# hzeller/timg

Measured on NVIDIA H100. Metric: Mpixels/s scale+dither+sixel-encode @4K→cell, higher is better.
Workload: dtype u8/f32

## Files before the change

### timg_b200/csrc/sixel_dither.cu

```cuda
#include <algorithm>
#include <cstdlib>

#include "sixel.cuh"

namespace b200timg {

#ifdef CUSIM
__device__ __forceinline__ uint32_t prmt(uint32_t a, uint32_t b, uint32_t s) { return __byte_perm(a, b, s); }
#else
__device__ __forceinline__ uint32_t prmt(uint32_t a, uint32_t b, uint32_t s) {
    uint32_t d;
    asm("prmt.b32 %0, %1, %2, %3;" : "=r"(d) : "r"(a), "r"(b), "r"(s));
    return d;
}
#endif

constexpr int D2_WMAX = 24;
constexpr int D2_CH = 16;
constexpr int D2_IN_STRIDE = D2_CH + 1;
constexpr int D2_OUT_STRIDE = 20;
constexpr int D2_WARP_SMEM = 2 * 32 * D2_IN_STRIDE * 4 + 32 * D2_OUT_STRIDE + D2_CH * 16;

struct TapW { uint32_t r, g, b; };

template <int K> __device__ __forceinline__ uint32_t tap_rg(const TapW &t) {
    constexpr uint32_t sel = (uint32_t)K | ((8u | K) << 4) | ((4u + K) << 8) | ((8u | (4u + K)) << 12);
    return prmt(t.r, t.g, sel);
}
template <int K> __device__ __forceinline__ uint32_t tap_b(const TapW &t) {
    constexpr uint32_t sel = (uint32_t)K | ((8u | K) << 4) | (4u << 8) | (4u << 12);
    return prmt(t.b, 0u, sel);
}
__device__ __forceinline__ uint32_t add_clamp(uint32_t v, uint32_t t) { return __viaddmin_s16x2_relu(v, t, 0x00ff00ffu); }

struct Dither2Geom { int w, h, nb32, bands_per_cta, nwarps; unsigned spin_ns; };

struct DitherUniform {
    typedef Dither2Geom Params;
    const Dither2Geom &G; int f, g;
    __device__ __forceinline__ explicit DitherUniform(const Dither2Geom &p) : G(p), f(blockIdx.y), g(blockIdx.x) {}
    __device__ __forceinline__ int w() const { return G.w; }
    __device__ __forceinline__ int h() const { return G.h; }
    __device__ __forceinline__ int nb32() const { return G.nb32; }
    __device__ __forceinline__ int bands_per_cta() const { return G.bands_per_cta; }
    __device__ __forceinline__ int nwarps() const { return G.nwarps; }
    __device__ __forceinline__ unsigned spin_ns() const { return G.spin_ns; }
    __device__ __forceinline__ long long px0() const { return (long long)f * G.w * G.h; }
    __device__ __forceinline__ long long idx0() const { return (long long)f * G.w * G.h; }
    __device__ __forceinline__ long long bnd0() const { return (long long)f * G.nb32 * G.w; }
    __device__ __forceinline__ long long prog0() const { return (long long)f * G.nb32; }
};
struct DitherMixed {
    typedef MixedSixelParams Params;
    MixedSixelFrame D; int f, g, nw;
    __device__ __forceinline__ explicit DitherMixed(const MixedSixelParams &P) : nw(P.nwarps) {
        f = sixel_owner(P.cta_start, P.n_frames, blockIdx.x);
        g = (int)(blockIdx.x - P.cta_start[f]);
        D = P.desc[f];
    }
    __device__ __forceinline__ int w() const { return D.w; }
    __device__ __forceinline__ int h() const { return D.h; }
    __device__ __forceinline__ int nb32() const { return D.nb32; }
    __device__ __forceinline__ int bands_per_cta() const { return D.bands_per_cta; }
    __device__ __forceinline__ int nwarps() const { return nw; }
    __device__ __forceinline__ unsigned spin_ns() const { return 256; }
    __device__ __forceinline__ long long px0() const { return (long long)D.fb_px; }
    __device__ __forceinline__ long long idx0() const { return (long long)D.idx; }
    __device__ __forceinline__ long long bnd0() const { return (long long)D.bnd; }
    __device__ __forceinline__ long long prog0() const { return (long long)D.prog0; }
};

template <class A>
__global__ void __launch_bounds__(D2_WMAX * 32)
sixel_dither2_kernel(const uint32_t *__restrict__ fb, typename A::Params G, SixelWork W, uint4 *__restrict__ bnd_all, int *__restrict__ gprog_all) {
    extern __shared__ __align__(16) uint8_t s_dyn2[];
    __shared__ uint2 s_pal2[256];
    __shared__ uint32_t s_tap[512];
    __shared__ volatile int s_progress[2048];
    const A a(G);
    const int f = a.f, g = a.g;
    const SixelFrameHdr *hdr = W.hdr + f;
    if (!hdr->diffuse) return;
    const int tid = threadIdx.x, lane = tid & 31, wid = tid >> 5;
    const int nthreads = a.nwarps() * 32, w = a.w(), h = a.h();
    uint8_t *s_lut = s_dyn2;
    for (int i = tid; i < 32768 / 16; i += nthreads)
        reinterpret_cast<uint4 *>(s_lut)[i] = reinterpret_cast<const uint4 *>(W.lut + (long long)f * 32768)[i];
    for (int i = tid; i < 256; i += nthreads) {
        const uint32_t p = hdr->palette[i];
        s_pal2[i] = make_uint2((256u - (p & 0xff)) | ((256u - ((p >> 8) & 0xff)) << 16), (256u - ((p >> 16) & 0xff)) | (256u << 16));
    }
    for (int i = tid; i < 512; i += nthreads) {
        const int e = i - 256;
        const int t7 = e * 7 / 16, t3 = e * 3 / 16, t5 = e * 5 / 16, t1 = e / 16;
        s_tap[i] = (uint32_t)(t7 & 0xff) | ((uint32_t)(t3 & 0xff) << 8) | ((uint32_t)(t5 & 0xff) << 16) | ((uint32_t)(t1 & 0xff) << 24);
    }
    const int band_lo = g * a.bands_per_cta(), band_hi = min(a.nb32(), band_lo + a.bands_per_cta());
    const int nlocal = band_hi - band_lo;
    for (int i = tid; i < nlocal; i += nthreads) s_progress[i] = 0;
    __syncthreads();
    uint32_t *s_in = reinterpret_cast<uint32_t *>(s_dyn2 + 32768 + (size_t)wid * D2_WARP_SMEM);
    uint8_t *s_out = reinterpret_cast<uint8_t *>(s_in + 2 * 32 * D2_IN_STRIDE);
    uint4 *s_bnd = reinterpret_cast<uint4 *>(s_out + 32 * D2_OUT_STRIDE);
    const uint32_t *frame = fb + a.px0();
    uint8_t *index = W.index + a.idx0();
    uint4 *bnd = bnd_all + a.bnd0();
    volatile int *gprog = gprog_all + a.prog0();
    const int hrow = lane >> 4, hcol = lane & 15;
    const int qrow = lane >> 3, qcol = lane & 7;
    const bool even_w = (w & 1) == 0;
    const TapW Z = {0u, 0u, 0u};

    for (int band = band_lo + wid; band < band_hi; band += a.nwarps()) {
        const int lb = band - band_lo;
        const int y = band * 32 + lane;
        const bool row_ok = y < h, last_row = (y == h - 1);
        const bool prev_remote = band > 0 && lb == 0;
        const bool publish_remote = band + 1 < a.nb32() && band + 1 == band_hi;
        const uint4 *bin = band > 0 ? bnd + (long long)(band - 1) * w : nullptr;
        uint4 *bout = bnd + (long long)band * w;
        TapW own = Z, a0 = Z, a1 = Z, a2 = Z, e_first = Z;
        const int steps = w + 62, nchunks = (steps + D2_CH - 1) / D2_CH;
        uint32_t pre[16];
        auto load_chunk = [&](int c) {
            if (even_w) {
#pragma unroll
                for (int i = 0; i < 8; ++i) {
                    const int r = 4 * i + qrow, yy = band * 32 + r, x = c * D2_CH - 2 * r + 2 * qcol;
                    uint2 v = make_uint2(0u, 0u);
                    if (yy < h && x >= 0 && x < w) v = *reinterpret_cast<const uint2 *>(frame + (long long)yy * w + x);
                    pre[2 * i] = v.x; pre[2 * i + 1] = v.y;
                }
            } else {
#pragma unroll
                for (int i = 0; i < 16; ++i) {
                    const int r = 2 * i + hrow, yy = band * 32 + r, x = c * D2_CH - 2 * r + hcol;
                    pre[i] = (yy < h && x >= 0 && x < w) ? frame[(long long)yy * w + x] : 0u;
                }
            }
        };
        auto store_chunk = [&](int c) {
            uint32_t *t = s_in + (c & 1) * 32 * D2_IN_STRIDE;
            if (even_w) {
#pragma unroll
                for (int i = 0; i < 8; ++i) {
                    uint32_t *q = t + (4 * i + qrow) * D2_IN_STRIDE + 2 * qcol;
                    q[0] = pre[2 * i]; q[1] = pre[2 * i + 1];
                }
            } else {
#pragma unroll
                for (int i = 0; i < 16; ++i) t[(2 * i + hrow) * D2_IN_STRIDE + hcol] = pre[i];
            }
        };
        load_chunk(0); store_chunk(0);
        __syncwarp();
        for (int c = 0; c < nchunks; ++c) {
            const int t0 = c * D2_CH;
            if (c + 1 < nchunks) load_chunk(c + 1);
            if (band > 0) {
                const int need = min(w, t0 + D2_CH + 1);
                if (lane == 0) {
                    if (prev_remote) { while (gprog[band - 1] < need) __nanosleep(a.spin_ns()); __threadfence(); }
                    else { while (s_progress[lb - 1] < need) __nanosleep(a.spin_ns()); __threadfence_block(); }
                }
                __syncwarp();
                const int bx = t0 + 1 + lane;
                if (lane < D2_CH) s_bnd[lane] = bx < w ? __ldcg(bin + bx) : make_uint4(0u, 0u, 0u, 0u);
                if (c == 0 && lane == 0) { const uint4 q = __ldcg(bin); a0.r = q.x; a0.g = q.y; a0.b = q.z; }
                __syncwarp();
            }
            const uint32_t *tin = s_in + (c & 1) * 32 * D2_IN_STRIDE + lane * D2_IN_STRIDE;
            const bool interior = (t0 - 62 >= 1) && (t0 + D2_CH - 1 <= w - 2) && (band * 32 + 31 < h - 1);
            if (interior) {
#pragma unroll 4
                for (int j = 0; j < D2_CH; ++j) {
                    TapW n;
                    n.r = __shfl_up_sync(0xffffffffu, own.r, 1); n.g = __shfl_up_sync(0xffffffffu, own.g, 1); n.b = __shfl_up_sync(0xffffffffu, own.b, 1);
                    if (lane == 0) { if (band > 0) { const uint4 q = s_bnd[j]; n.r = q.x; n.g = q.y; n.b = q.z; } else n = Z; }
                    a2 = a1; a1 = a0; a0 = n;
                    const uint32_t px = tin[j];
                    uint32_t vrg = prmt(px, 0u, 0x4140u), vb = prmt(px, 0u, 0x4442u);
                    vrg = add_clamp(vrg, tap_rg<3>(a2)); vb = add_clamp(vb, tap_b<3>(a2));
                    vrg = add_clamp(vrg, tap_rg<2>(a1)); vb = add_clamp(vb, tap_b<2>(a1));
                    vrg = add_clamp(vrg, tap_rg<1>(a0)); vb = add_clamp(vb, tap_b<1>(a0));
                    vrg = add_clamp(vrg, tap_rg<0>(own)); vb = add_clamp(vb, tap_b<0>(own));
                    const uint32_t cell = ((vrg & 0xf8u) << 7) | ((vrg >> 14) & 0x3e0u) | (vb >> 3);
                    const uint32_t ci = s_lut[cell];
                    const uint2 np = s_pal2[ci];
                    const uint32_t erg = vrg + np.x, eb = vb + np.y;
                    own.r = s_tap[erg & 0x1ffu]; own.g = s_tap[erg >> 16]; own.b = s_tap[eb & 0x1ffu];
                    s_out[lane * D2_OUT_STRIDE + j] = (uint8_t)ci;
                    if (lane == 31) __stcg(bout + (t0 + j - 62), make_uint4(own.r, own.g, own.b, 0u));
                }
            } else {
#pragma unroll 2
                for (int j = 0; j < D2_CH; ++j) {
                    const int t = t0 + j, x = t - 2 * lane;
                    TapW n;
                    n.r = __shfl_up_sync(0xffffffffu, own.r, 1); n.g = __shfl_up_sync(0xffffffffu, own.g, 1); n.b = __shfl_up_sync(0xffffffffu, own.b, 1);
                    if (lane == 0) { if (band > 0) { const uint4 q = s_bnd[j]; n.r = q.x; n.g = q.y; n.b = q.z; } else n = Z; }
                    a2 = a1; a1 = a0; a0 = n;
                    uint32_t ci = 0;
                    if (x >= 0 && x < w && row_ok) {
                        const uint32_t px = tin[j];
                        uint32_t vrg = prmt(px, 0u, 0x4140u), vb = prmt(px, 0u, 0x4442u);
                        vrg = add_clamp(vrg, tap_rg<3>(a2)); vb = add_clamp(vb, tap_b<3>(a2));
                        vrg = add_clamp(vrg, tap_rg<2>(a1)); vb = add_clamp(vb, tap_b<2>(a1));
                        vrg = add_clamp(vrg, tap_rg<1>(a0)); vb = add_clamp(vb, tap_b<1>(a0));
                        if (x == w - 1) { vrg = add_clamp(vrg, tap_rg<1>(e_first)); vb = add_clamp(vb, tap_b<1>(e_first)); }
                        vrg = add_clamp(vrg, tap_rg<0>(own)); vb = add_clamp(vb, tap_b<0>(own));
                        const uint32_t cell = ((vrg & 0xf8u) << 7) | ((vrg >> 14) & 0x3e0u) | (vb >> 3);
                        ci = s_lut[cell];
                        if (x < w - 1 && !last_row) {
                            const uint2 np = s_pal2[ci];
                            const uint32_t erg = vrg + np.x, eb = vb + np.y;
                            own.r = s_tap[erg & 0x1ffu]; own.g = s_tap[erg >> 16]; own.b = s_tap[eb & 0x1ffu];
                        } else {
                            own = Z;
                        }
                        if (x == 0) e_first = own;
                        if (lane == 31) __stcg(bout + x, make_uint4(own.r, own.g, own.b, 0u));
                    } else if (x >= w) {
                        own = Z;
                    }
                    s_out[lane * D2_OUT_STRIDE + j] = (uint8_t)ci;
                }
            }
            __syncwarp();
            if (even_w) {
#pragma unroll
                for (int i = 0; i < 8; ++i) {
                    const int r = 4 * i + qrow, yy = band * 32 + r, x = t0 - 2 * r + 2 * qcol;
                    if (yy < h && x >= 0 && x < w)
                        *reinterpret_cast<unsigned short *>(index + (long long)yy * w + x) =
                            *reinterpret_cast<const unsigned short *>(s_out + r * D2_OUT_STRIDE + 2 * qcol);
                }
            } else {
#pragma unroll
                for (int i = 0; i < 16; ++i) {
                    const int r = 2 * i + hrow, yy = band * 32 + r, x = t0 - 2 * r + hcol;
                    if (yy < h && x >= 0 && x < w) index[(long long)yy * w + x] = s_out[r * D2_OUT_STRIDE + hcol];
                }
            }
            {
                const int done = min(w, t0 + D2_CH - 62);
                if (lane == 31 && done > 0) {
                    if (publish_remote) { __threadfence(); gprog[band] = done; }
                    __threadfence_block();
                    s_progress[lb] = done;
                }
            }
            if (c + 1 < nchunks) store_chunk(c + 1);
            __syncwarp();
        }
    }
}

size_t sixel_dither_workspace(int w, int h, int n_frames, size_t *o_bnd, size_t *o_prog) {
    const size_t nb32 = (size_t)(h + 31) / 32;
    size_t off = 0;
    *o_bnd = off; off += (sizeof(uint4) * nb32 * (size_t)w * n_frames + 255) / 256 * 256;
    *o_prog = off; off += (sizeof(int) * nb32 * n_frames + 255) / 256 * 256;
    return off;
}

SixelDitherShape sixel_dither_shape(int nb32, int n_frames, int n_total, int sm_count, bool env) {
    SixelDitherShape S;
    int per_frame = 1;
    if (n_total < sm_count) {
        per_frame = std::max(1, std::min(sm_count / n_total, (nb32 + 7) / 8));
        if (const char *e = env ? getenv("B200TIMG_DITHER_SPLIT") : nullptr) per_frame = std::max(1, std::min(atoi(e), nb32));
        if ((long long)per_frame * n_frames > sm_count) per_frame = std::max(1, sm_count / n_frames);
    }
    S.bands_per_cta = (nb32 + per_frame - 1) / per_frame;
    S.per_frame = (nb32 + S.bands_per_cta - 1) / S.bands_per_cta;
    int wmax = D2_WMAX;
    if (const char *e = env ? getenv("B200TIMG_DITHER_WARPS") : nullptr) wmax = std::max(1, std::min(atoi(e), D2_WMAX));
    S.rounds = (S.bands_per_cta + wmax - 1) / wmax;
    S.nwarps = (S.bands_per_cta + S.rounds - 1) / S.rounds;
    return S;
}

int launch_sixel_dither(b200timg_ctx *ctx, const uint32_t *fb, int w, int h, int n_frames, int n_total, const SixelWork &W, void *d_bnd, void *d_prog) {
    Dither2Geom G;
    G.w = w; G.h = h; G.nb32 = (h + 31) / 32;
    G.spin_ns = 256;
    if (const char *e = getenv("B200TIMG_DITHER_SPIN")) G.spin_ns = (unsigned)std::max(0, std::min(atoi(e), 100000));
    const SixelDitherShape S = sixel_dither_shape(G.nb32, n_frames, n_total, ctx->sm_count, true);
    const int per_frame = S.per_frame;
    G.bands_per_cta = S.bands_per_cta;
    G.nwarps = S.nwarps;
    const size_t smem = 32768 + (size_t)G.nwarps * D2_WARP_SMEM;
    B2_CUDA(ctx, cudaFuncSetAttribute(sixel_dither2_kernel<DitherUniform>, cudaFuncAttributeMaxDynamicSharedMemorySize, 32768 + D2_WMAX * D2_WARP_SMEM));
    if (per_frame > 1) B2_CUDA(ctx, cudaMemsetAsync(d_prog, 0, sizeof(int) * (size_t)G.nb32 * n_frames, ctx->stream));
    B2_KERNEL(ctx, "sixel_dither2_kernel");
    sixel_dither2_kernel<DitherUniform><<<dim3(per_frame, n_frames), G.nwarps * 32, smem, ctx->stream>>>(fb, G, W, static_cast<uint4 *>(d_bnd), static_cast<int *>(d_prog));
    B2_LAUNCH_CHECK(ctx);
    return B200TIMG_OK;
}

int launch_sixel_dither_mixed(b200timg_ctx *ctx, const uint32_t *fb, unsigned n_ctas, const MixedSixelParams &M, const SixelWork &W,
                              void *d_bnd, void *d_prog, size_t n_prog, bool split) {
    const size_t smem = 32768 + (size_t)M.nwarps * D2_WARP_SMEM;
    B2_CUDA(ctx, cudaFuncSetAttribute(sixel_dither2_kernel<DitherMixed>, cudaFuncAttributeMaxDynamicSharedMemorySize, 32768 + D2_WMAX * D2_WARP_SMEM));
    if (split) B2_CUDA(ctx, cudaMemsetAsync(d_prog, 0, sizeof(int) * n_prog, ctx->stream));
    B2_KERNEL(ctx, "sixel_dither2_mixed_kernel");
    sixel_dither2_kernel<DitherMixed><<<n_ctas, M.nwarps * 32, smem, ctx->stream>>>(fb, M, W, static_cast<uint4 *>(d_bnd), static_cast<int *>(d_prog));
    B2_LAUNCH_CHECK(ctx);
    return B200TIMG_OK;
}

}
```

Baseline: 75790.

## Reorder dither chunk pipeline and stage boundary stores through shared memory

Moves the next-chunk global load after the neighbor-band wait. Lane 31 now stages boundary error terms in a per-warp shared buffer, and 16 lanes write them to global in one coalesced burst. The index write-back moves after progress publication, so downstream bands are unblocked sooner, and the interior loop packs four palette indices per 32-bit shared store. Palette and tap tables move into dynamic shared memory. Optional clock instrumentation is added behind a compile flag, at the cost of slightly more shared memory per warp.

```diff
diff --git a/timg_b200/csrc/sixel_dither.cu b/timg_b200/csrc/sixel_dither.cu
--- a/timg_b200/csrc/sixel_dither.cu
+++ b/timg_b200/csrc/sixel_dither.cu
@@ -19,7 +19,8 @@
 constexpr int D2_CH = 16;
 constexpr int D2_IN_STRIDE = D2_CH + 1;
 constexpr int D2_OUT_STRIDE = 20;
-constexpr int D2_WARP_SMEM = 2 * 32 * D2_IN_STRIDE * 4 + 32 * D2_OUT_STRIDE + D2_CH * 16;
+constexpr int D2_WARP_SMEM = 2 * 32 * D2_IN_STRIDE * 4 + 32 * D2_OUT_STRIDE + 2 * D2_CH * 16;
+constexpr int D2_TABLES = 32768 + 2048 + 2048;
 
 struct TapW { uint32_t r, g, b; };
 
@@ -32,6 +33,7 @@
     return prmt(t.b, 0u, sel);
 }
 __device__ __forceinline__ uint32_t add_clamp(uint32_t v, uint32_t t) { return __viaddmin_s16x2_relu(v, t, 0x00ff00ffu); }
+
 
 struct Dither2Geom { int w, h, nb32, bands_per_cta, nwarps; unsigned spin_ns; };
 
@@ -70,17 +72,33 @@
     __device__ __forceinline__ long long prog0() const { return (long long)D.prog0; }
 };
 
+#ifdef B200TIMG_DITHER_CLOCKS
+enum { DCLK_SETUP, DCLK_WAIT, DCLK_FETCH, DCLK_STEPS, DCLK_STAGE, DCLK_PHASES };
+__device__ unsigned long long g_dither_clocks[DCLK_PHASES + 1];
+#define DCLK_BEGIN unsigned dclk_[DCLK_PHASES] = {}, dclk_steps_ = 0; unsigned dclk_t_ = (unsigned)clock()
+#define DCLK(k) do { const unsigned t_ = (unsigned)clock(); dclk_[k] += t_ - dclk_t_; dclk_t_ = t_; } while (0)
+#define DCLK_STEP(n) (dclk_steps_ += (n))
+#define DCLK_END() do { if ((threadIdx.x & 31) == 0) { for (int k_ = 0; k_ < DCLK_PHASES; ++k_) \
+        atomicAdd(&g_dither_clocks[k_], (unsigned long long)dclk_[k_]); atomicAdd(&g_dither_clocks[DCLK_PHASES], (unsigned long long)dclk_steps_); } } while (0)
+#else
+#define DCLK_BEGIN do {} while (0)
+#define DCLK(k) do {} while (0)
+#define DCLK_STEP(n) do {} while (0)
+#define DCLK_END() do {} while (0)
+#endif
+
 template <class A>
 __global__ void __launch_bounds__(D2_WMAX * 32)
 sixel_dither2_kernel(const uint32_t *__restrict__ fb, typename A::Params G, SixelWork W, uint4 *__restrict__ bnd_all, int *__restrict__ gprog_all) {
     extern __shared__ __align__(16) uint8_t s_dyn2[];
-    __shared__ uint2 s_pal2[256];
-    __shared__ uint32_t s_tap[512];
+    uint2 *s_pal2 = reinterpret_cast<uint2 *>(s_dyn2 + 32768);
+    uint32_t *s_tap = reinterpret_cast<uint32_t *>(s_dyn2 + 32768 + 2048);
     __shared__ volatile int s_progress[2048];
     const A a(G);
     const int f = a.f, g = a.g;
     const SixelFrameHdr *hdr = W.hdr + f;
     if (!hdr->diffuse) return;
+    DCLK_BEGIN;
     const int tid = threadIdx.x, lane = tid & 31, wid = tid >> 5;
     const int nthreads = a.nwarps() * 32, w = a.w(), h = a.h();
     uint8_t *s_lut = s_dyn2;
@@ -99,9 +117,11 @@
     const int nlocal = band_hi - band_lo;
     for (int i = tid; i < nlocal; i += nthreads) s_progress[i] = 0;
     __syncthreads();
-    uint32_t *s_in = reinterpret_cast<uint32_t *>(s_dyn2 + 32768 + (size_t)wid * D2_WARP_SMEM);
+    DCLK(DCLK_SETUP);
+    uint32_t *s_in = reinterpret_cast<uint32_t *>(s_dyn2 + D2_TABLES + (size_t)wid * D2_WARP_SMEM);
     uint8_t *s_out = reinterpret_cast<uint8_t *>(s_in + 2 * 32 * D2_IN_STRIDE);
     uint4 *s_bnd = reinterpret_cast<uint4 *>(s_out + 32 * D2_OUT_STRIDE);
+    uint4 *s_bo = s_bnd + D2_CH;
     const uint32_t *frame = fb + a.px0();
     uint8_t *index = W.index + a.idx0();
     uint4 *bnd = bnd_all + a.bnd0();
@@ -156,7 +176,7 @@
         __syncwarp();
         for (int c = 0; c < nchunks; ++c) {
             const int t0 = c * D2_CH;
-            if (c + 1 < nchunks) load_chunk(c + 1);
+            DCLK(DCLK_STAGE);
             if (band > 0) {
                 const int need = min(w, t0 + D2_CH + 1);
                 if (lane == 0) {
@@ -164,14 +184,18 @@
                     else { while (s_progress[lb - 1] < need) __nanosleep(a.spin_ns()); __threadfence_block(); }
                 }
                 __syncwarp();
+                DCLK(DCLK_WAIT);
                 const int bx = t0 + 1 + lane;
                 if (lane < D2_CH) s_bnd[lane] = bx < w ? __ldcg(bin + bx) : make_uint4(0u, 0u, 0u, 0u);
                 if (c == 0 && lane == 0) { const uint4 q = __ldcg(bin); a0.r = q.x; a0.g = q.y; a0.b = q.z; }
                 __syncwarp();
-            }
+                DCLK(DCLK_FETCH);
+            }
+            if (c + 1 < nchunks) load_chunk(c + 1);
             const uint32_t *tin = s_in + (c & 1) * 32 * D2_IN_STRIDE + lane * D2_IN_STRIDE;
             const bool interior = (t0 - 62 >= 1) && (t0 + D2_CH - 1 <= w - 2) && (band * 32 + 31 < h - 1);
             if (interior) {
+                uint32_t ob = 0;
 #pragma unroll 4
                 for (int j = 0; j < D2_CH; ++j) {
                     TapW n;
@@ -189,8 +213,9 @@
                     const uint2 np = s_pal2[ci];
                     const uint32_t erg = vrg + np.x, eb = vb + np.y;
                     own.r = s_tap[erg & 0x1ffu]; own.g = s_tap[erg >> 16]; own.b = s_tap[eb & 0x1ffu];
-                    s_out[lane * D2_OUT_STRIDE + j] = (uint8_t)ci;
-                    if (lane == 31) __stcg(bout + (t0 + j - 62), make_uint4(own.r, own.g, own.b, 0u));
+                    ob |= ci << (8 * (j & 3));
+                    if ((j & 3) == 3) { *reinterpret_cast<uint32_t *>(s_out + lane * D2_OUT_STRIDE + j - 3) = ob; ob = 0; }
+                    if (lane == 31) s_bo[j] = make_uint4(own.r, own.g, own.b, 0u);
                 }
             } else {
 #pragma unroll 2
@@ -219,7 +244,7 @@
                             own = Z;
                         }
                         if (x == 0) e_first = own;
-                        if (lane == 31) __stcg(bout + x, make_uint4(own.r, own.g, own.b, 0u));
+                        if (lane == 31) s_bo[j] = make_uint4(own.r, own.g, own.b, 0u);
                     } else if (x >= w) {
                         own = Z;
                     }
@@ -227,21 +252,11 @@
                 }
             }
             __syncwarp();
-            if (even_w) {
-#pragma unroll
-                for (int i = 0; i < 8; ++i) {
-                    const int r = 4 * i + qrow, yy = band * 32 + r, x = t0 - 2 * r + 2 * qcol;
-                    if (yy < h && x >= 0 && x < w)
-                        *reinterpret_cast<unsigned short *>(index + (long long)yy * w + x) =
-                            *reinterpret_cast<const unsigned short *>(s_out + r * D2_OUT_STRIDE + 2 * qcol);
-                }
-            } else {
-#pragma unroll
-                for (int i = 0; i < 16; ++i) {
-                    const int r = 2 * i + hrow, yy = band * 32 + r, x = t0 - 2 * r + hcol;
-                    if (yy < h && x >= 0 && x < w) index[(long long)yy * w + x] = s_out[r * D2_OUT_STRIDE + hcol];
-                }
-            }
+            if (lane < D2_CH && band * 32 + 31 < h) {
+                const int x = t0 + lane - 62;
+                if (x >= 0 && x < w) __stcg(bout + x, s_bo[lane]);
+            }
+            __syncwarp();
             {
                 const int done = min(w, t0 + D2_CH - 62);
                 if (lane == 31 && done > 0) {
@@ -250,10 +265,28 @@
                     s_progress[lb] = done;
                 }
             }
+            DCLK(DCLK_STEPS); DCLK_STEP(D2_CH);
+            if (even_w) {
+#pragma unroll
+                for (int i = 0; i < 8; ++i) {
+                    const int r = 4 * i + qrow, yy = band * 32 + r, x = t0 - 2 * r + 2 * qcol;
+                    if (yy < h && x >= 0 && x < w)
+                        *reinterpret_cast<unsigned short *>(index + (long long)yy * w + x) =
+                            *reinterpret_cast<const unsigned short *>(s_out + r * D2_OUT_STRIDE + 2 * qcol);
+                }
+            } else {
+#pragma unroll
+                for (int i = 0; i < 16; ++i) {
+                    const int r = 2 * i + hrow, yy = band * 32 + r, x = t0 - 2 * r + hcol;
+                    if (yy < h && x >= 0 && x < w) index[(long long)yy * w + x] = s_out[r * D2_OUT_STRIDE + hcol];
+                }
+            }
             if (c + 1 < nchunks) store_chunk(c + 1);
             __syncwarp();
         }
     }
+    DCLK(DCLK_STAGE);
+    DCLK_END();
 }
 
 size_t sixel_dither_workspace(int w, int h, int n_frames, size_t *o_bnd, size_t *o_prog) {
@@ -290,8 +323,8 @@
     const int per_frame = S.per_frame;
     G.bands_per_cta = S.bands_per_cta;
     G.nwarps = S.nwarps;
-    const size_t smem = 32768 + (size_t)G.nwarps * D2_WARP_SMEM;
-    B2_CUDA(ctx, cudaFuncSetAttribute(sixel_dither2_kernel<DitherUniform>, cudaFuncAttributeMaxDynamicSharedMemorySize, 32768 + D2_WMAX * D2_WARP_SMEM));
+    const size_t smem = D2_TABLES + (size_t)G.nwarps * D2_WARP_SMEM;
+    B2_CUDA(ctx, cudaFuncSetAttribute(sixel_dither2_kernel<DitherUniform>, cudaFuncAttributeMaxDynamicSharedMemorySize, D2_TABLES + D2_WMAX * D2_WARP_SMEM));
     if (per_frame > 1) B2_CUDA(ctx, cudaMemsetAsync(d_prog, 0, sizeof(int) * (size_t)G.nb32 * n_frames, ctx->stream));
     B2_KERNEL(ctx, "sixel_dither2_kernel");
     sixel_dither2_kernel<DitherUniform><<<dim3(per_frame, n_frames), G.nwarps * 32, smem, ctx->stream>>>(fb, G, W, static_cast<uint4 *>(d_bnd), static_cast<int *>(d_prog));
@@ -301,8 +334,8 @@
 
 int launch_sixel_dither_mixed(b200timg_ctx *ctx, const uint32_t *fb, unsigned n_ctas, const MixedSixelParams &M, const SixelWork &W,
                               void *d_bnd, void *d_prog, size_t n_prog, bool split) {
-    const size_t smem = 32768 + (size_t)M.nwarps * D2_WARP_SMEM;
-    B2_CUDA(ctx, cudaFuncSetAttribute(sixel_dither2_kernel<DitherMixed>, cudaFuncAttributeMaxDynamicSharedMemorySize, 32768 + D2_WMAX * D2_WARP_SMEM));
+    const size_t smem = D2_TABLES + (size_t)M.nwarps * D2_WARP_SMEM;
+    B2_CUDA(ctx, cudaFuncSetAttribute(sixel_dither2_kernel<DitherMixed>, cudaFuncAttributeMaxDynamicSharedMemorySize, D2_TABLES + D2_WMAX * D2_WARP_SMEM));
     if (split) B2_CUDA(ctx, cudaMemsetAsync(d_prog, 0, sizeof(int) * n_prog, ctx->stream));
     B2_KERNEL(ctx, "sixel_dither2_mixed_kernel");
     sixel_dither2_kernel<DitherMixed><<<n_ctas, M.nwarps * 32, smem, ctx->stream>>>(fb, M, W, static_cast<uint4 *>(d_bnd), static_cast<int *>(d_prog));
@@ -311,3 +344,14 @@
 }
 
 }
+
+#ifdef B200TIMG_DITHER_CLOCKS
+extern "C" int b200timg_dither_clocks(unsigned long long *out) {
+    using b200timg::g_dither_clocks;
+    static const unsigned long long zero[b200timg::DCLK_PHASES + 1] = {};
+    if (cudaDeviceSynchronize() != cudaSuccess || cudaMemcpyFromSymbol(out, g_dither_clocks, sizeof zero) != cudaSuccess ||
+        cudaMemcpyToSymbol(g_dither_clocks, zero, sizeof zero) != cudaSuccess)
+        return -3;
+    return 0;
+}
+#endif
```

Result: faster. 77580, median of 6 (+2.4%).
